# vismaychuriwala/Fast-Image-Editing-with-Generative-Models

Measured on AMD Instinct MI355X. Metric: PIE-Bench images/sec @1024^2 SSD-1B fp16 4-step, higher is better.
Workload: dtype f16

## Files before the change

### fast-image-editing-with-generative-models_amd/csrc/conv_halo.hip

```cpp
#include "gemm_common.h"

using namespace fie_gemm;

namespace {

constexpr int HP = 18;
constexpr int HPIECES = (HP * HP + 7) / 8;
constexpr int HALO_B = HPIECES * 1024;
constexpr int HSLOTS = 6;
constexpr int BNH = 128;
constexpr int STH = 3;
constexpr int WSTAGE_B = BNH * 128;
constexpr int WRING_OFF = 0;
constexpr int HALO_OFF = STH * WSTAGE_B;
constexpr int DUMP_OFF = HALO_OFF + 2 * HALO_B;
constexpr int kLdsHalo = DUMP_OFF + 1024;
constexpr int RWH = BNH / 64;

constexpr int n_w(bool last, int t) { return last && t + 2 > 8 ? 0 : RWH; }
constexpr int n_h(bool last, int t) { return !last && t < HSLOTS ? 1 : 0; }
constexpr int n_wait(bool last, int t) { return (t > 0 ? n_h(last, t - 1) : 0) + n_w(last, t) + n_h(last, t); }

template <bool STAMP>
__global__ __launch_bounds__(512) void conv_halo_kernel(GemmArgs p) {
    constexpr int FM = 4, FN = 4, WM = 64, WN = 64;
    extern __shared__ __attribute__((aligned(16))) half_t smem[];
    char* const lds = reinterpret_cast<char*>(smem);

    const int tid = threadIdx.x;
    const int lane = tid & 63;
    const int wave = __builtin_amdgcn_readfirstlane(tid >> 6);
    const int grp = wave >> 2;
    const int wm = wave & 3, wn = wave >> 2;

    const int bid = xcd_remap(blockIdx.x, gridDim.x);
    const int nt = bid % p.nbn, patch = bid / p.nbn;
    const int ppr = p.OW >> 4, ppi = (p.OH >> 4) * ppr;
    const int b = patch / ppi, pr = patch - b * ppi;
    const int py = pr / ppr, px = pr - py * ppr;
    const int y0 = py << 4, x0 = px << 4;
    const int m0 = (b * p.OH + y0) * p.OW + x0, n0 = nt * BNH;

    const int live = p.probe == 1 ? 0 : 1;
    const __amdgpu_buffer_rsrc_t rs_a = buf_rsrc(p.A1, (int)p.a1_bytes * live);
    const __amdgpu_buffer_rsrc_t rs_w = buf_rsrc(p.Wt, (int)p.w_bytes * live);

    unsigned h_off[HSLOTS];
#pragma unroll
    for (int i = 0; i < HSLOTS; ++i) {
        const int q = wave + 8 * i;
        const int pl = q * 8 + (lane >> 3);
        const int hy = pl / HP, hx = pl - hy * HP;
        const int iy = y0 + hy - 1, ix = x0 + hx - 1;
        const bool ok = q < HPIECES && pl < HP * HP && iy >= 0 && iy < p.H && ix >= 0 && ix < p.W;
        const unsigned chunk = (unsigned)((lane & 7) ^ (hx & 7));
        h_off[i] = ok ? ((unsigned)(b * p.H + iy) * (unsigned)p.W + (unsigned)ix) * (unsigned)p.Cin * 2u + chunk * 16u : kOob;
    }
    auto halo_dst = [&](int i, int buf) -> half_t* {
        const int q = wave + 8 * i;
        return reinterpret_cast<half_t*>(lds + (q < HPIECES ? HALO_OFF + buf * HALO_B + q * 1024 : DUMP_OFF));
    };
    const int lr = lane >> 3;
    const unsigned w_base = (unsigned)(n0 + wave * 8 + lr) * (unsigned)p.ldw * 2u + (unsigned)((lane & 7) ^ lr) * 16u;
    const unsigned w_step = 64u * (unsigned)p.ldw * 2u;
    auto issue_w = [&](int stage, unsigned soff) {
#pragma unroll
        for (int i = 0; i < RWH; ++i)
            bload16(rs_w, reinterpret_cast<half_t*>(lds + WRING_OFF + stage * WSTAGE_B + (wave + 8 * i) * 1024), w_base + (unsigned)i * w_step, soff);
    };
    const unsigned cin2 = (unsigned)p.Cin * 2u;

    const int fr = lane & 15, fq = lane >> 4;
    unsigned a_rd[3][2];
#pragma unroll
    for (int kx = 0; kx < 3; ++kx)
#pragma unroll
        for (int kh = 0; kh < 2; ++kh)
            a_rd[kx][kh] = (unsigned)((wm * FM * HP + fr + kx) * 128 + (((kh * 4 + fq) ^ ((fr + kx) & 7)) << 4));
    unsigned w_rd[2];
#pragma unroll
    for (int kh = 0; kh < 2; ++kh) w_rd[kh] = (unsigned)(2 * lds_off(wn * WN + fr, kh * 4 + fq));

    f32x4 acc[FN][FM];
#pragma unroll
    for (int i = 0; i < FN; ++i)
#pragma unroll
        for (int j = 0; j < FM; ++j) acc[i][j] = (f32x4){0.f, 0.f, 0.f, 0.f};

    unsigned seg[8] = {0, 0, 0, 0, 0, 0, 0, 0}, tprev = 0;
    auto stamp = [&](int i) {
        if constexpr (STAMP) {
            __builtin_amdgcn_sched_barrier(0);
            const unsigned t = (unsigned)__builtin_amdgcn_s_memtime();
            seg[i] += t - tprev;
            tprev = t;
            __builtin_amdgcn_sched_barrier(0);
        }
    };
    if constexpr (STAMP) tprev = (unsigned)__builtin_amdgcn_s_memtime();

    const int nchunks = p.Cin / BK;
#pragma unroll
    for (int i = 0; i < HSLOTS; ++i) bload16(rs_a, halo_dst(i, 0), h_off[i], 0u);
    issue_w(0, 0u);
    issue_w(1, nchunks * 9 > 1 ? cin2 : 0u);
    wait_vm_barrier<RWH>();
    if (grp == 1) __builtin_amdgcn_s_barrier();
    stamp(5);

    f16x8 fw[2][FN], fa[2][FM];
    auto kstep = [&](auto lastc, auto tapc, int c, unsigned hb) {
        constexpr bool LAST = decltype(lastc)::value;
        constexpr int T = decltype(tapc)::value;
        constexpr int KY = T / 3, KX = T % 3;
        constexpr int STAGE = T % STH, FILL = (T + 2) % STH;
        if constexpr (n_w(LAST, T) > 0) {
            constexpr int T2 = (T + 2) % 9;
            const int c2 = T + 2 > 8 ? c + 1 : c;
            issue_w(FILL, (unsigned)T2 * cin2 + (unsigned)c2 * (BK * 2));
        }
        if constexpr (n_h(LAST, T) > 0) bload16(rs_a, halo_dst(T, (c + 1) & 1), h_off[T], (unsigned)(c + 1) * (BK * 2));
        stamp(0);
        const char* const hal = lds + HALO_OFF + hb;
        const char* const wst = lds + WRING_OFF + STAGE * WSTAGE_B;
#pragma unroll
        for (int kh = 0; kh < 2; ++kh) {
#pragma unroll
            for (int i = 0; i < FN; ++i) fw[kh][i] = *reinterpret_cast<const f16x8*>(wst + w_rd[kh] + i * 16 * 128);
#pragma unroll
            for (int j = 0; j < FM; ++j) fa[kh][j] = *reinterpret_cast<const f16x8*>(hal + a_rd[KX][kh] + (j + KY) * HP * 128);
        }
        asm volatile("s_waitcnt lgkmcnt(0)" ::: "memory");
        stamp(1);
        wait_vm_barrier<n_wait(LAST, T)>();
        stamp(2);
        __builtin_amdgcn_sched_barrier(0);
        __builtin_amdgcn_s_setprio(1);
#pragma unroll
        for (int kh = 0; kh < 2; ++kh)
#pragma unroll
            for (int i = 0; i < FN; ++i)
#pragma unroll
                for (int j = 0; j < FM; ++j) acc[i][j] = __builtin_amdgcn_mfma_f32_16x16x32_f16(fw[kh][i], fa[kh][j], acc[i][j], 0, 0, 0);
        __builtin_amdgcn_s_setprio(0);
        __builtin_amdgcn_sched_barrier(0);
        stamp(3);
        __builtin_amdgcn_s_barrier();
        stamp(4);
    };
    auto chunk = [&](auto lastc, int c) {
        const unsigned hb = (c & 1) ? (unsigned)HALO_B : 0u;
        kstep(lastc, std::integral_constant<int, 0>{}, c, hb);
        kstep(lastc, std::integral_constant<int, 1>{}, c, hb);
        kstep(lastc, std::integral_constant<int, 2>{}, c, hb);
        kstep(lastc, std::integral_constant<int, 3>{}, c, hb);
        kstep(lastc, std::integral_constant<int, 4>{}, c, hb);
        kstep(lastc, std::integral_constant<int, 5>{}, c, hb);
        kstep(lastc, std::integral_constant<int, 6>{}, c, hb);
        kstep(lastc, std::integral_constant<int, 7>{}, c, hb);
        kstep(lastc, std::integral_constant<int, 8>{}, c, hb);
    };
    for (int c = 0; c + 1 < nchunks; ++c) chunk(std::false_type{}, c);
    chunk(std::true_type{}, nchunks - 1);
    if (grp == 0) __builtin_amdgcn_s_barrier();

    epilogue<FM, FN, WM, WN, true, true>(p, acc, m0, n0, wm, wn, lane);
    if constexpr (STAMP) {
        asm volatile("s_waitcnt vmcnt(0)" ::: "memory");
        stamp(6);
        if (p.stamps && lane == 0) {
#pragma unroll
            for (int i = 0; i < 8; ++i) p.stamps[((size_t)bid * 8 + wave) * 8 + i] = seg[i];
        }
    }
}


constexpr int K_FIRST = 0, K_MID = 1, K_LAST_F = 2, K_LAST_N = 3, K_LASTREG_S = 4;
constexpr int n2_w(int kind, int t) { return kind == K_LAST_N && t + 2 > 8 ? 0 : RWH; }
constexpr int n2_h(int kind, int t) { return kind != K_LAST_N && t < HSLOTS ? 1 : 0; }
constexpr int n2_st(int var, int kind, int t) { return kind == K_FIRST && t < 8 ? ((var & 2) ? 1 : 2) : 0; }
constexpr int n2_tail(bool res, int kind, int t) { return n2_h(kind, t); }
constexpr int n2_wait(int var, bool res, int kind, int t) {
    return (t > 0 ? n2_tail(res, kind, t - 1) : 0) + ((var & 8) ? 0 : n2_w(kind, t) + n2_tail(res, kind, t));
}
static_assert(n2_tail(true, K_LAST_F, 8) == 0 && n2_tail(true, K_FIRST, 8) == 0 && n2_st(0, K_FIRST, 8) == 0, "tap 8 carries nothing behind its weights");

// ... 587 lines not shown
                }
                su = row16_sum(su);
                sq = row16_sum(sq);
                if (gn_sh >= 3) {
                    float a0 = su, b0 = su, a1 = sq, b1 = sq;
                    asm volatile("s_nop 1\n\tv_permlane16_swap_b32 %0, %1" : "+v"(a0), "+v"(b0));
                    asm volatile("s_nop 1\n\tv_permlane16_swap_b32 %0, %1" : "+v"(a1), "+v"(b1));
                    su = a0 + b0; sq = a1 + b1;
                }
                if (gn_sh >= 4) {
                    float a0 = su, b0 = su, a1 = sq, b1 = sq;
                    asm volatile("s_nop 1\n\tv_permlane32_swap_b32 %0, %1" : "+v"(a0), "+v"(b0));
                    asm volatile("s_nop 1\n\tv_permlane32_swap_b32 %0, %1" : "+v"(a1), "+v"(b1));
                    su = a0 + b0; sq = a1 + b1;
                }
                const int rows_per_group = 1 << (gn_sh - 2);
                const bool ok = fr == 0 && (fq & (rows_per_group - 1)) == 0;
                const unsigned slot = gslot_prev + (unsigned)(JJ * (p.OW >> 4) * p.gn_G) + (unsigned)(((wn * WN + I * 16) >> gn_sh) + (fq >> (gn_sh - 2)));
                u32x2 bits;
                const float2 v2 = make_float2(su, sq);
                __builtin_memcpy(&bits, &v2, 8);
                __builtin_amdgcn_raw_buffer_store_b64(bits, rs_g, ok ? slot * 8u : kOob, 0, 0);
            }, std::make_integer_sequence<int, (FM / 2) * FN>{});
        }
#pragma unroll
        for (int jj = 0; jj < FM / 2; ++jj)
#pragma unroll
            for (int i = 0; i < FN; ++i) {
                u32x4 v = {outp[i][2 * jj][0], outp[i][2 * jj][1], outp[i][2 * jj + 1][0], outp[i][2 * jj + 1][1]};
                if constexpr (DEFER) {
                    asm volatile("s_nop 1\n\tv_permlane16_swap_b32 %0, %1" : "+v"(v[0]), "+v"(v[2]));
                    asm volatile("s_nop 1\n\tv_permlane16_swap_b32 %0, %1" : "+v"(v[1]), "+v"(v[3]));
                }
                __builtin_amdgcn_raw_buffer_store_b128(v, rs_c, edge_off(ro_prev + (unsigned)(2 * jj) * c_jstep + (unsigned)(i * 32), 2 * jj), 0, 0);
            }
    } else {
#pragma unroll
        for (int j = 0; j < FM; ++j)
#pragma unroll
            for (int i = 0; i < FN; ++i) __builtin_amdgcn_raw_buffer_store_b64(outp[i][j], rs_c, ro_prev + (unsigned)j * c_jstep + (unsigned)(i * 32), 0, 0);
    }
    if constexpr (STAMP) {
        asm volatile("s_waitcnt vmcnt(0)" ::: "memory");
        stamp(6);
        if (p.stamps && lane == 0) {
#pragma unroll
            for (int i = 0; i < 8; ++i) p.stamps[((size_t)bid * 8 + wave) * 12 + i] = seg[i];
#pragma unroll
            for (int i = 0; i < 4; ++i) p.stamps[((size_t)bid * 8 + wave) * 12 + 8 + i] = kseg[i];
        }
    }
}

template <bool RES, bool GN, bool RB, int VAR, bool STAMP, bool SIDE = false, bool GNA = false, bool EDGE = false>
hipError_t halo2_attr() {
    return hipFuncSetAttribute(reinterpret_cast<const void*>(&conv_halo2_kernel<RES, GN, RB, VAR, STAMP, SIDE, GNA, EDGE>), hipFuncAttributeMaxDynamicSharedMemorySize, kLdsHalo);
}

}

int fie_conv_halo_init(void) {
    hipError_t e = hipFuncSetAttribute(reinterpret_cast<const void*>(&conv_halo_kernel<false>), hipFuncAttributeMaxDynamicSharedMemorySize, kLdsHalo);
    if (e == hipSuccess) e = hipFuncSetAttribute(reinterpret_cast<const void*>(&conv_halo_kernel<true>), hipFuncAttributeMaxDynamicSharedMemorySize, kLdsHalo);
    if (e == hipSuccess) e = halo2_attr<false, false, false, 6, false>();
    if (e == hipSuccess) e = halo2_attr<false, true, false, 6, false>();
    if (e == hipSuccess) e = halo2_attr<true, false, false, 6, false>();
    if (e == hipSuccess) e = halo2_attr<true, true, false, 6, false>();
    if (e == hipSuccess) e = halo2_attr<false, false, true, 6, false>();
    if (e == hipSuccess) e = halo2_attr<false, true, true, 6, false>();
    if (e == hipSuccess) e = halo2_attr<false, false, false, 0, false>();
    if (e == hipSuccess) e = halo2_attr<false, true, false, 0, false>();
    if (e == hipSuccess) e = halo2_attr<true, false, false, 0, false>();
    if (e == hipSuccess) e = halo2_attr<true, true, false, 0, false>();
    if (e == hipSuccess) e = halo2_attr<false, false, true, 0, false>();
    if (e == hipSuccess) e = halo2_attr<false, true, true, 0, false>();
    if (e == hipSuccess) e = halo2_attr<false, false, false, 6, true>();
    if (e == hipSuccess) e = hipFuncSetAttribute(reinterpret_cast<const void*>(&conv_halo2_kernel<false, false, false, 6, false, true>), hipFuncAttributeMaxDynamicSharedMemorySize, kLdsHalo);
    if (e == hipSuccess) e = hipFuncSetAttribute(reinterpret_cast<const void*>(&conv_halo2_kernel<false, true, false, 6, false, true>), hipFuncAttributeMaxDynamicSharedMemorySize, kLdsHalo);
    if (e == hipSuccess) e = halo2_attr<true, true, false, 6, true>();
    if (e == hipSuccess) e = hipFuncSetAttribute(reinterpret_cast<const void*>(&conv_halo2_kernel<false, true, false, 6, false, false, true>), hipFuncAttributeMaxDynamicSharedMemorySize, kLdsHalo + 8192);
    if (e == hipSuccess) e = hipFuncSetAttribute(reinterpret_cast<const void*>(&conv_halo2_kernel<true, true, false, 6, false, false, true>), hipFuncAttributeMaxDynamicSharedMemorySize, kLdsHalo + 8192);
    if (e == hipSuccess) e = halo2_attr<false, false, false, 6, false, false, false, true>();
    if (e == hipSuccess) e = halo2_attr<true, false, false, 6, false, false, false, true>();
    if (e == hipSuccess) e = halo2_attr<false, false, true, 6, false, false, false, true>();
    if (e == hipSuccess) e = halo2_attr<false, false, false, 6, false, true, false, true>();
    if (e != hipSuccess) {
        fie_set_error("conv_halo: hipFuncSetAttribute failed: %s", hipGetErrorString(e));
        return FIE_EHIP;
    }
    return FIE_OK;
}

bool fie_conv_halo_ok(const GemmArgs& a) {
    const bool base = a.stride == 1 && !a.ups && !a.taps2 && !a.oscat && a.pt == 1 && a.pl == 1 && a.H == a.OH && a.W == a.OW && a.OH % 16 == 0 &&
                      a.OW % 16 == 0 && a.Cin % BK == 0 && a.Cin >= BK && !a.w_scale && !a.out_f8 && a.splitk <= 1;
    if (!base) return false;
    if (!a.A2) return !a.A3 && a.K == 9 * a.Cin;
    return a.C2x % BK == 0 && a.C3x % BK == 0 && a.C2x > 0 && (a.A3 != nullptr) == (a.C3x > 0) && a.K == 9 * a.Cin + a.C2x + a.C3x && a.Cin >= 2 * BK && a.N % BNH == 0 &&
           !a.res && !a.rowbias && a.act == FIE_ACT_NONE && a.scale == 1.f && a.lda2 * 2 * (int64_t)a.OW * a.OH < (1ll << 31) && a.lda3 * 2 * (int64_t)a.OW * a.OH < (1ll << 31);
}

bool fie_conv_halo_edge_ok(const GemmArgs& a) {
    const bool base = a.stride == 1 && !a.ups && !a.taps2 && !a.oscat && a.pt == 1 && a.pl == 1 && a.H == a.OH && a.W == a.OW && a.OH > 0 && a.OW > 0 &&
                      (a.OH % 16 != 0 || a.OW % 16 != 0) && a.M % (a.OH * a.OW) == 0 && a.Cin % BK == 0 && a.Cin >= 2 * BK && !a.w_scale && !a.out_f8 &&
                      a.splitk <= 1 && a.N % 64 == 0 && a.ldc >= a.N && !a.gn_partial && !a.gna_tab && a.act == FIE_ACT_NONE && a.scale == 1.f && !(a.rowbias && a.res);
    if (!base) return false;
    if (!a.A2) return !a.A3 && a.K == 9 * a.Cin;
    return a.C2x % BK == 0 && a.C3x % BK == 0 && a.C2x > 0 && (a.A3 != nullptr) == (a.C3x > 0) && a.K == 9 * a.Cin + a.C2x + a.C3x && !a.res && !a.rowbias &&
           a.lda2 * 2 * (int64_t)a.OW * a.OH < (1ll << 31) && a.lda3 * 2 * (int64_t)a.OW * a.OH < (1ll << 31);
}

int64_t fie_conv_halo_patches(const GemmArgs& a) {
    if (a.OH <= 0 || a.OW <= 0) return 0;
    return (int64_t)(a.M / (a.OH * a.OW)) * ((a.OH + 15) / 16) * ((a.OW + 15) / 16);
}

bool fie_conv_halo_gna_ok(const GemmArgs& a) {
    if (!fie_conv_halo_ok(a) || a.A2 || a.rowbias) return false;
    const int nbn = (a.N + BNH - 1) / BNH;
    return a.M == a.OH * a.OW && a.Cin >= 2 * BK && a.Cin <= 1024 && a.N % BNH == 0 && nbn <= 64 && a.act == FIE_ACT_NONE && a.scale == 1.f && a.gn_partial != nullptr &&
           (a.gn_cg == 4 || a.gn_cg == 8 || a.gn_cg == 16);
}

int fie_launch_conv_halo(fie_ctx* ctx, GemmArgs& a, int variant) {
    if (variant == 6) {
        FIE_REQUIRE(fie_conv_halo_edge_ok(a), "halo-resident conv with edge patches (tile code 78): stride-1 same-size 3x3 conv with H or W %% 16 != 0, Cin %% 64 == 0, "
                    "Cin >= 128, N %% 64 == 0, no activation / scale / GroupNorm sums only");
        a.frag_ld = a.OW;
        a.nbn = (a.N + BNH - 1) / BNH;
        a.nbm = (int)fie_conv_halo_patches(a);
        const int tiles = a.nbm * a.nbn;
        int g = tiles < ctx->num_cus ? tiles : ctx->num_cus;
        g -= g % a.nbn;
        FIE_REQUIRE(g >= a.nbn && a.nbn <= ctx->num_cus, "halo-resident conv: more column tiles than CUs");
        const dim3 grid((unsigned)g);
        if (a.A2) fie_launch(ctx, (conv_halo2_kernel<false, false, false, 6, false, true, false, true>), grid, dim3(512), kLdsHalo, a);
        else if (a.res) fie_launch(ctx, (conv_halo2_kernel<true, false, false, 6, false, false, false, true>), grid, dim3(512), kLdsHalo, a);
        else if (a.rowbias) fie_launch(ctx, (conv_halo2_kernel<false, false, true, 6, false, false, false, true>), grid, dim3(512), kLdsHalo, a);
        else fie_launch(ctx, (conv_halo2_kernel<false, false, false, 6, false, false, false, true>), grid, dim3(512), kLdsHalo, a);
        FIE_LAUNCH_CHECK();
        return FIE_OK;
    }
    FIE_REQUIRE(fie_conv_halo_ok(a), "halo-resident conv: stride-1 same-size 3x3 conv with H, W %% 16 == 0 and Cin %% 64 == 0 only");
    a.frag_ld = a.OW;
    a.nbn = (a.N + BNH - 1) / BNH;
    a.nbm = (a.M / (a.OH * a.OW)) * (a.OH >> 4) * (a.OW >> 4);
    const int tiles = a.nbm * a.nbn;
    const bool side = a.A2 != nullptr;
    FIE_REQUIRE(!(side && variant != 2), "halo-resident conv: 1x1 side inputs run on tile code 72 only");
    if (a.gna_tab) {
        FIE_REQUIRE(fie_conv_halo_gna_ok(a), "halo-resident conv with the input's GroupNorm applied in LDS: shape or epilogue not built (fie_conv3x3_gn_ok)");
        int g = tiles < ctx->num_cus ? tiles : ctx->num_cus;
        g -= g % a.nbn;
        const int lds_bytes = kLdsHalo + a.Cin * 8;
        if (a.res) fie_launch(ctx, (conv_halo2_kernel<true, true, false, 6, false, false, true>), dim3((unsigned)g), dim3(512), lds_bytes, a);
        else fie_launch(ctx, (conv_halo2_kernel<false, true, false, 6, false, false, true>), dim3((unsigned)g), dim3(512), lds_bytes, a);
        FIE_LAUNCH_CHECK();
        return FIE_OK;
    }
    if (!side && variant >= 2 && tiles <= ctx->num_cus) variant = variant == 4 ? 1 : 0;
    if (!side && variant >= 2 && (a.Cin < 2 * BK || a.N % BNH != 0 || (a.rowbias && a.res) || (variant == 4 && a.rowbias) || a.act != FIE_ACT_NONE || a.scale != 1.f)) variant = variant == 4 ? 1 : 0;
    if (variant < 2) {
        const dim3 grid((unsigned)tiles);
        if (variant == 1) fie_launch(ctx, (conv_halo_kernel<true>), grid, dim3(512), kLdsHalo, a);
        else fie_launch(ctx, (conv_halo_kernel<false>), grid, dim3(512), kLdsHalo, a);
        FIE_LAUNCH_CHECK();
        return FIE_OK;
    }
    int g = tiles < ctx->num_cus ? tiles : ctx->num_cus;
    g -= g % a.nbn;
    FIE_REQUIRE(g >= a.nbn && a.nbn <= ctx->num_cus, "halo-resident conv: more column tiles than CUs");
    const dim3 grid((unsigned)g);
    const bool res = a.res != nullptr, gn = a.gn_partial != nullptr, rb = a.rowbias != nullptr;
    FIE_REQUIRE(!gn || a.gn_cg == 4 || a.gn_cg == 8 || a.gn_cg == 16, "halo-resident conv: GroupNorm sums need 4, 8 or 16 channels per group");
#define FIE_HALO2(RES, GN, RB, VAR, ST) fie_launch(ctx, (conv_halo2_kernel<RES, GN, RB, VAR, ST>), grid, dim3(512), kLdsHalo, a)
#define FIE_HALO2_V(VAR)                                                                   \
    do {                                                                                   \
        if (rb && gn) FIE_HALO2(false, true, true, VAR, false);                            \
        else if (rb) FIE_HALO2(false, false, true, VAR, false);                            \
        else if (res && gn) FIE_HALO2(true, true, false, VAR, false);                      \
        else if (res) FIE_HALO2(true, false, false, VAR, false);                           \
        else if (gn) FIE_HALO2(false, true, false, VAR, false);                            \
        else FIE_HALO2(false, false, false, VAR, false);                                   \
    } while (0)
    if (side) { if (gn) fie_launch(ctx, (conv_halo2_kernel<false, true, false, 6, false, true>), grid, dim3(512), kLdsHalo, a); else fie_launch(ctx, (conv_halo2_kernel<false, false, false, 6, false, true>), grid, dim3(512), kLdsHalo, a); }
    else if (variant == 4) { if (res || gn) FIE_HALO2(true, true, false, 6, true); else FIE_HALO2(false, false, false, 6, true); }
    else if (variant == 5) FIE_HALO2_V(0);
    else FIE_HALO2_V(6);
#undef FIE_HALO2_V
#undef FIE_HALO2
    FIE_LAUNCH_CHECK();
    return FIE_OK;
}
```

### fast-image-editing-with-generative-models_amd/csrc/fie_internal.h

```cpp
#pragma once
#include <hip/hip_runtime.h>
#include <stdint.h>
#include <stdio.h>
#include <string.h>
#include <map>
#include <string>
#include <tuple>
#include <utility>
#include <vector>
#include "../../include/fie.h"

typedef _Float16 half_t;
typedef _Float16 f16x8 __attribute__((ext_vector_type(8)));
typedef _Float16 f16x4 __attribute__((ext_vector_type(4)));
typedef _Float16 f16x2 __attribute__((ext_vector_type(2)));
typedef float f32x4 __attribute__((ext_vector_type(4)));
typedef short s16x4 __attribute__((ext_vector_type(4)));
typedef unsigned u32x4 __attribute__((ext_vector_type(4)));

struct fie_launch_rec {
    const void* fn;
    dim3 grid, block;
    unsigned lds;
    std::vector<unsigned char> blob;
// ... 1 lines not shown
};
struct fie_program {
    std::vector<fie_launch_rec> recs;
    hipEvent_t done = nullptr;
    hipStream_t last_stream = nullptr;
    bool has_done = false;
};

struct fie_weight { const void* ptr; int64_t n, ld; };
struct fie_step_cache { char* ptr; int64_t bytes; bool filled; };

struct fie_tile_override { int mode, M, N, K, code; };

struct fie_tune_key {
    int mode, M, N, K, K1, geom, w8;
    bool operator<(const fie_tune_key& o) const {
        return std::tie(mode, M, N, K, K1, geom, w8) < std::tie(o.mode, o.M, o.N, o.K, o.K1, o.geom, o.w8);
    }
};

struct fie_ctx {
    int device;
    hipStream_t stream;
    int num_cus;
    int force_tile = 0;
    int gemm_probe = 0;
    int epi_prefetch = 1;
    unsigned* gemm_stamps = nullptr;
    float* gn_target = nullptr;
    int64_t gn_target_rows = 0;
    int gn_target_groups = 0;
    int attn_variant = 0;
    int gn_onepass = 1;
    unsigned* err_flag = nullptr;
    void* sk_ws = nullptr;
    int64_t sk_bytes = 0;
    int splitk_mode = 1;
    int autotune = 0;
    std::map<fie_tune_key, int> tuned;
    int tune_exclude[16] = {0};
    void* tune_buf = nullptr;
    void* tune_flush = nullptr;
    size_t tune_bytes = 0;
    int n_overrides = 0;
    fie_tile_override overrides[32];
    char last_kernel[128] = "";
    fie_program* recording = nullptr;
    std::vector<std::string>* oplog = nullptr;
    char op_desc[384] = "";
    std::vector<std::string>* tune_cands = nullptr;
    std::map<std::string, fie_program*> graphs;
    std::map<std::string, fie_step_cache> step_caches;
    std::map<std::string, fie_weight> weights;
};

template <typename T>
inline void fie_pack_arg(fie_launch_rec& r, const T& v) {
    size_t off = (r.blob.size() + alignof(T) - 1) / alignof(T) * alignof(T);
    r.blob.resize(off + sizeof(T));
    memcpy(r.blob.data() + off, &v, sizeof(T));
    r.offs.push_back((unsigned)off);
}

void fie_oplog_append(fie_ctx* ctx, const void* fn, dim3 grid, dim3 block, unsigned lds);
#define FIE_DESC(ctx, ...)                                                              \
    do {                                                                                \
        if ((ctx)->oplog) snprintf((ctx)->op_desc, sizeof((ctx)->op_desc), __VA_ARGS__); \
    } while (0)

template <typename... KArgs, typename... Args>
inline void fie_launch(fie_ctx* ctx, void (*kernel)(KArgs...), dim3 grid, dim3 block, unsigned lds, Args&&... args) {
    static_assert(sizeof...(KArgs) == sizeof...(Args), "argument count");
    std::tuple<KArgs...> vals(static_cast<KArgs>(args)...);
    std::apply([&](const KArgs&... a) { hipLaunchKernelGGL(kernel, grid, block, lds, ctx->stream, a...); }, vals);
    if (ctx->oplog) fie_oplog_append(ctx, reinterpret_cast<const void*>(kernel), grid, block, lds);
    if (ctx->recording) {
        fie_launch_rec r;
        r.fn = reinterpret_cast<const void*>(kernel);
        r.grid = grid; r.block = block; r.lds = lds;
        std::apply([&](const KArgs&... a) { (fie_pack_arg(r, a), ...); }, vals);
        ctx->recording->recs.push_back(std::move(r));
    }
}

void fie_set_error(const char* fmt, ...);

#define FIE_REQUIRE(cond, ...)                         \
    do {                                               \
        if (!(cond)) {                                 \
            fie_set_error(__VA_ARGS__);                \
            return FIE_EINVAL;                         \
        }                                              \
    } while (0)

#define FIE_LAUNCH_CHECK()                                                         \
    do {                                                                           \
        hipError_t e__ = hipGetLastError();                                        \
        if (e__ != hipSuccess) {                                                   \
            fie_set_error("%s:%d launch failed: %s", __FILE__, __LINE__,           \
                          hipGetErrorString(e__));                                 \
            return FIE_EHIP;                                                       \
        }                                                                          \
    } while (0)

static inline int64_t fie_roundup(int64_t x, int64_t m) { return (x + m - 1) / m * m; }

// ... 36 lines not shown
```

### fast-image-editing-with-generative-models_amd/hip.py

```python
import ctypes
import os
import subprocess

import torch

from . import header

_CSRC = os.path.join(os.path.dirname(os.path.abspath(__file__)), "csrc")
LIB_PATH = os.environ.get("FIE_LIB_PATH") or os.path.join(_CSRC, "libfie_hip.so")

_P, _I, _F = ctypes.c_void_p, ctypes.c_int, ctypes.c_float

ACT_NONE, ACT_SILU, ACT_GELU, ACT_QUICK_GELU, ACT_GEGLU = (header.DEFINES["ACT_" + n] for n in ("NONE", "SILU", "GELU", "QUICK_GELU", "GEGLU"))
SIGNATURES = {name: args for name, (_, args) in header.FUNCTIONS.items()}

_lib = None


def build(force=False):
    if force:
        subprocess.run(["make", "-C", _CSRC, "clean"], check=True, capture_output=True)
    r = subprocess.run(["make", "-C", _CSRC, "-j4"], capture_output=True, text=True)
    if r.returncode != 0:
        raise RuntimeError("building libfie_hip.so failed:\n" + r.stdout[-4000:] + r.stderr[-4000:])
# ... 76 lines not shown
        assert name in GRAPH_NAMES, name
        _chk(lib().fie_graph_register(self.ctx.h, name.encode(), self.h))

    def close(self):
        if self.h:
            lib().fie_program_destroy(self.ctx.h, self.h)
            self.h = _P()


class W8:

    def __init__(self, q, scale):
        self.q, self.scale = q, scale

    def stride(self, d):
        return self.q.stride(d)

    def dequant(self):
        return self.q.view(torch.float8_e4m3fn).float() * self.scale[:, None]


class Context:

    def __init__(self, device=0, dtype=torch.float16):
        if dtype not in (torch.float16, torch.float32):
            raise ValueError(f"dtype {dtype} not supported (float16 or float32)")
        self.dtype = dtype
        self.f32 = dtype == torch.float32
        if not torch.cuda.is_available():
            raise RuntimeError("no HIP device visible: the fie_amd hot path has no CPU fallback")
        self.device = torch.device("cuda", device)
        h = _P()
        _chk(lib().fie_ctx_create(device, None, ctypes.byref(h)))
        self.h = h
        self._err = torch.zeros(4, device=self.device, dtype=torch.int32)
        self._err_host = torch.zeros(4, dtype=torch.int32).pin_memory()
        _chk(lib().fie_ctx_error_flag(self.h, self._err.data_ptr()))
        self._stream = None
        self._gn_ws = {}
        self._gn_stats = {}
        self._gn_gen = 0
        self._sk_ws = {}
        self._sk_bound = None
        self._sk_pinned = False
        self._cap_stream = None
        self._prog_ws = []
        self.splitk_bytes = int(os.environ.get("FIE_SPLITK_MB", "96")) << 20
        self.gn_from_epilogue = os.environ.get("FIE_GN_FROM_EPILOGUE", "1") != "0"
        self.gn_quads = os.environ.get("FIE_GN_QUADS", "1") != "0"
        self._epi_prefetch = True
        self.up2x_parity = os.environ.get("FIE_UP2X_PARITY", "1") != "0"
        self.ln_fold = os.environ.get("FIE_LN_FOLD", "1") != "0"
        self.kv_group = os.environ.get("FIE_KV_GROUP", "1") != "0"
        self.ln_fold_which = os.environ.get("FIE_LN_FOLD_WHICH", "qkv,q2")
        self.ln_fold_ff1 = os.environ.get("FIE_LN_FOLD_FF1", "0") != "0"
        self.conv_plus_shortcut = os.environ.get("FIE_CONV_PLUS", "1") != "0"
        self._resize_tables = {}
        self.ws_tag = 0
        self._keep = None
        self.w8 = False
        self.a8 = os.environ.get("FIE_A8", "1") != "0"
        self.gn_fuse_conv = os.environ.get("FIE_GN_FUSE_CONV", "0") == "1"
        self.calib = False
        self.tune_frozen = os.environ.get("FIE_TUNE_FROZEN", "0") == "1"
        self.tune_table_entries = 0
        self.load_tune_table()

    def fetch_device_errors(self):
        self._err_host.copy_(self._err, non_blocking=True)

    def check_device_errors(self, fetch=True):
        if fetch:
            self.fetch_device_errors()
            torch.cuda.current_stream(self.device).synchronize()
        code = int(self._err_host[0])
        if code:
            self._err.zero_()
            self._err_host.zero_()
            what = {1: "fie_time_embed_f16: the in-launch barrier timed out (a workgroup never arrived); the timestep embedding of that "
                       "launch is invalid"}.get(code, "unknown device error")
            raise FieError(f"device error {code}: {what}")

    def sync_stream(self):
        s = torch.cuda.current_stream(self.device).cuda_stream
        if s != self._stream:
            _chk(lib().fie_ctx_set_stream(self.h, s))
            self._stream = s

    def load_tune_table(self, path=None):
        path = path or os.environ.get("FIE_TUNE_TABLE")
        if not path or self.f32:
            return 0
        with open(path) as f:
            n = lib().fie_gemm_autotune_load(self.h, f.read().encode())
        if n < 0:
            raise FieError(f"fie_gemm_autotune_load: {lib().fie_last_error().decode()}")
        self.tune_table_entries = n
        return n

    def _bind_splitk(self):
        if self._sk_pinned or self.f32 or not self.splitk_bytes:
            return
        key = (self._stream, self.ws_tag)
        if key == self._sk_bound:
            return
        ws = self._sk_ws.get(key)
# ... 5 lines not shown
    def capture_stream(self):
        if self._cap_stream is None:
            self._cap_stream = torch.cuda.Stream(device=self.device)
        with torch.cuda.stream(self._cap_stream):
            self.sync_stream()
            self._bind_splitk()
        torch.cuda.synchronize(self.device)
        return self._cap_stream

    def splitk_counters_clear(self):
        torch.cuda.synchronize(self.device)
        live = list(self._sk_ws.values()) + [w for w in (r() for r in self._prog_ws) if w is not None]
        return all(int(ws[:16384].view(torch.int32).abs().max()) == 0 for ws in live)

    def record(self):
        import contextlib

        @contextlib.contextmanager
        def cm():
            prog = Program(self)
            self.sync_stream()
            own = None
            if not self.f32 and self.splitk_bytes:
                own = torch.zeros(self.splitk_bytes, device=self.device, dtype=torch.uint8)
                prog.keep.append(own)
                import weakref
                self._prog_ws = [r for r in self._prog_ws if r() is not None] + [weakref.ref(own)]
                _chk(lib().fie_splitk_workspace(self.h, own.data_ptr(), own.numel()))
                self._sk_pinned = True
            _chk(lib().fie_program_begin(self.h, ctypes.byref(prog.h)))
            self._keep = prog.keep
            try:
                yield prog
            finally:
                self._keep = None
                _chk(lib().fie_program_end(self.h))
                if own is not None:
                    self._sk_pinned = False
                    self._sk_bound = None
        return cm()

    def run_named(self, name):
        self.sync_stream()
        _chk(getattr(lib(), "fie_" + name)(self.h))

    def _alloc(self, shape, dtype=None, zero=False):
        t = (torch.zeros if zero else torch.empty)(shape, device=self.device, dtype=dtype or self.dtype)
        if self._keep is not None:
            self._keep.append(t)
        return t

    def force_tile(self, code):
        _chk(lib().fie_debug_force_tile(self.h, int(code)))

    def prefetch(self, t, stream=None, blocks=16):
        _chk(lib().fie_prefetch(self.h, t.data_ptr(), t.numel() * t.element_size(), stream.cuda_stream if stream is not None else None, int(blocks)))

    def autotune(self, on=True):
        _chk(lib().fie_gemm_autotune(self.h, int(on)))

    def tune_exclude(self, codes):
        return lib().fie_debug_tune_exclude(self.h, (codes or "").encode())

    def autotune_report(self):
        buf = ctypes.create_string_buffer(1 << 20)
        n = lib().fie_gemm_autotune_report(self.h, buf, len(buf))
        return n, buf.value.decode()

    def splitk(self, on=True):
        _chk(lib().fie_debug_splitk(self.h, int(bool(on))))

    def oplog(self, on=True):
        _chk(lib().fie_debug_oplog(self.h, int(on)))
        self._oplog_on = bool(on)

    def oplog_mark(self, text):
        if getattr(self, "_oplog_on", False):
            _chk(lib().fie_debug_oplog_mark(self.h, text.encode()))

    def oplog_read(self):
        n = lib().fie_debug_oplog_read(self.h, None, 0)
        buf = ctypes.create_string_buffer(int(n) + 16)
        lib().fie_debug_oplog_read(self.h, buf, len(buf))
        return [l for l in buf.value.decode().split("\n") if l]

    def tune_candidates(self, on=True):
        _chk(lib().fie_debug_tune_candidates(self.h, int(on)))

    def tune_candidates_read(self):
        n = lib().fie_debug_tune_candidates_read(self.h, None, 0)
        buf = ctypes.create_string_buffer(int(n) + 16)
        lib().fie_debug_tune_candidates_read(self.h, buf, len(buf))
        out = []
        for line in buf.value.decode().split("\n"):
            if line:
                key, rest = line.split(" rule=")
                rule, cands = rest.split(" cands=")
                out.append((key, int(rule), [int(c) for c in cands.split(",") if c]))
        return out

    def gemm_stamps(self, buf):
        _chk(lib().fie_debug_gemm_stamps(self.h, buf.data_ptr() if buf is not None else None))

    def gemm_probe(self, mode):
        _chk(lib().fie_debug_gemm_probe(self.h, int(mode)))

# ... 693 lines not shown
```

### include/fie.h

```cpp
#ifndef FIE_H_
#define FIE_H_

#include <stdint.h>

#ifdef __cplusplus
extern "C" {
#endif

#define FIE_OK 0
#define FIE_EINVAL (-1)
#define FIE_EHIP (-2)
#define FIE_ENODEV (-3)

#define FIE_DEVERR_TIME_EMBED_BARRIER 1u

#define FIE_ACT_NONE 0
#define FIE_ACT_SILU 1
#define FIE_ACT_GELU 2
#define FIE_ACT_QUICK_GELU 3
#define FIE_ACT_GEGLU 4

typedef struct fie_ctx fie_ctx;

int fie_version(void);
// ... 173 lines not shown
                           int64_t rows_per_image, int groups, const void* gamma, const void* beta, float eps,
                           int silu, void* workspace);
int fie_layernorm_f32(fie_ctx* ctx, const void* X, int64_t ldx, void* Y, int64_t ldy, int64_t rows, int C,
                      const void* gamma, const void* beta, float eps);
int fie_sinusoid_f32(fie_ctx* ctx, const float* vals, int B, int nvals, int dim, void* out, int64_t ld_out, int col0);
int fie_clip_embed_f32(fie_ctx* ctx, const int32_t* ids, int B, int T, int C, const void* tok_table,
                       const void* pos_table, void* out);
int fie_pixels_in_u8_f32(fie_ctx* ctx, const uint8_t* src, int H, int W, int normalize, void* dst, int copies);
int fie_pixels_out_f32_u8(fie_ctx* ctx, const void* src, int64_t ld_in, int H, int W, uint8_t* dst);
int fie_latent_prep_f32(fie_ctx* ctx, const void* moments, const float* eps_post, const float* noise, int64_t HW,
                        float scaling_factor, float sqrt_ab, float sqrt_1mab, float* latents_out, void* model_in,
                        int copies);
int fie_lcm_step_f32(fie_ctx* ctx, const void* eps, int64_t ld_eps, int nb, float guidance, float* latents,
                     const float* noise, int64_t HW, float sqrt_ab_t, float sqrt_1mab_t, float c_skip, float c_out,
                     float sqrt_ab_prev, float sqrt_1mab_prev, void* model_in, int copies, float inv_scaling,
                     void* decode_in);

int fie_debug_force_tile(fie_ctx* ctx, int tile);
int fie_debug_tile_override(fie_ctx* ctx, const char* spec);
int fie_conv3x3_plus_nhwc_f16(fie_ctx* ctx, const void* X, int B, int H, int W, int Cin, const void* Wpacked, int64_t ldw, void* Y, int64_t ldc, int Cout,
                              const void* bias, const void* rowbias, int64_t ld_rowbias, float scale, int act, const void* X2, int64_t ld2, int C2,
                              const void* X3, int64_t ld3, int C3);

int fie_conv_up2x_nhwc_f16(fie_ctx* ctx, const void* X, int B, int H, int W, int Cin, const void* W4, int64_t ldw, int Npad, void* Y, int64_t ldc,
                           int Cout, const void* bias, const void* rowbias, int64_t ld_rowbias, float scale, int act);

int fie_gn_stats_target(fie_ctx* ctx, void* partial, int64_t rows_per_image, int groups);
int fie_groupnorm_coef_f16(fie_ctx* ctx, int C, int B, int64_t rows_per_image, int groups, const void* gamma, const void* beta, float eps, const void* partial,
                           void* workspace, int partial_groups, float* coef);
int fie_conv3x3_gn_ok(fie_ctx* ctx, int B, int H, int W, int Cin, int Cout, int out_groups);
int fie_conv3x3_gn_nhwc_f16(fie_ctx* ctx, const void* X, int B, int H, int W, int Cin, const float* coef, int silu, const void* Wpacked, int64_t ldw, void* Y,
                            int64_t ldc, int Cout, const void* bias, const void* residual, int64_t ldr);
int64_t fie_gn_stats_bytes(int B, int64_t rows_per_image, int groups);
int fie_groupnorm_stats_nhwc_f16(fie_ctx* ctx, const void* X, int C, void* Y, int B, int64_t rows_per_image, int groups, const void* gamma,
                                 const void* beta, float eps, int silu, const void* partial, void* workspace, int partial_groups);

int fie_prefetch(fie_ctx* ctx, const void* ptr, int64_t bytes, void* stream, int blocks);
int fie_splitk_workspace(fie_ctx* ctx, void* workspace, int64_t bytes);
int fie_debug_splitk(fie_ctx* ctx, int mode);
int fie_gemm_autotune(fie_ctx* ctx, int on);
int fie_gemm_autotune_report(fie_ctx* ctx, char* buf, int cap);
int fie_gemm_autotune_load(fie_ctx* ctx, const char* text);
int fie_debug_tune_exclude(fie_ctx* ctx, const char* codes);
int fie_debug_gemm_probe(fie_ctx* ctx, int mode);
int fie_debug_epilogue_prefetch(fie_ctx* ctx, int on);
int fie_debug_gemm_stamps(fie_ctx* ctx, void* buf);
const char* fie_debug_last_gemm_kernel(fie_ctx* ctx);
int fie_debug_oplog(fie_ctx* ctx, int on);
int fie_debug_oplog_mark(fie_ctx* ctx, const char* text);
int64_t fie_debug_oplog_read(fie_ctx* ctx, char* buf, int64_t cap);
int fie_debug_tune_candidates(fie_ctx* ctx, int on);
int64_t fie_debug_tune_candidates_read(fie_ctx* ctx, char* buf, int64_t cap);
int fie_debug_attn_variant(fie_ctx* ctx, int variant);
int fie_debug_gn_onepass(fie_ctx* ctx, int enable);

int fie_canny_rgb_u8(const uint8_t* rgb, int H, int W, int low, int high, uint8_t* edges_rgb);

int64_t fie_canny_workspace_bytes(int H, int W);
int fie_canny_rgb_device_u8(fie_ctx* ctx, const uint8_t* rgb, int H, int W, int low, int high, void* workspace,
                            uint8_t* edges_rgb, int* iterations);
int fie_canny_rgb_device_begin_u8(fie_ctx* ctx, const uint8_t* rgb, int H, int W, int low, int high, int rounds, void* workspace, uint8_t* edges_rgb,
                                  int* host_flags);
int fie_canny_rgb_device_finish_u8(fie_ctx* ctx, int H, int W, void* workspace, uint8_t* edges_rgb, int* host_flags, int* iterations);

int fie_resize_rgb_u8(fie_ctx* ctx, const uint8_t* src, int H, int W, uint8_t* dst, int OH, int OW, const int* kx,
                      const int* bx, int ksx, const int* ky, const int* by, int ksy, uint8_t* tmp);

int fie_resize_l_u8(fie_ctx* ctx, const uint8_t* src, int H, int W, uint8_t* dst, int OH, int OW, const int* kx,
                    const int* bx, int ksx, const int* ky, const int* by, int ksy, uint8_t* tmp);

int fie_mask_prep(fie_ctx* ctx, const uint8_t* mask_l, int H, int W, const float* taps, int radius, float* mask_px,
                  uint8_t* mask_lat);
int fie_latent_prep_src(fie_ctx* ctx, const void* moments, const float* eps_post, const float* noise, int64_t HW,
                        float scaling_factor, float sqrt_ab, float sqrt_1mab, float* latents_out, void* model_in,
                        int copies, float* z0_out);
int fie_latent_prep_src_f32(fie_ctx* ctx, const void* moments, const float* eps_post, const float* noise, int64_t HW,
                            float scaling_factor, float sqrt_ab, float sqrt_1mab, float* latents_out, void* model_in,
                            int copies, float* z0_out);
int fie_lcm_step_masked(fie_ctx* ctx, const void* eps, int64_t ld_eps, int nb, float guidance, float* latents,
                        const float* noise, int64_t HW, float sqrt_ab_t, float sqrt_1mab_t, float c_skip, float c_out,
                        float sqrt_ab_prev, float sqrt_1mab_prev, void* model_in, int copies, float inv_scaling,
                        void* decode_in, const uint8_t* mask_lat, const float* z0, const float* noise_init);
int fie_lcm_step_masked_f32(fie_ctx* ctx, const void* eps, int64_t ld_eps, int nb, float guidance, float* latents,
                            const float* noise, int64_t HW, float sqrt_ab_t, float sqrt_1mab_t, float c_skip, float c_out,
                            float sqrt_ab_prev, float sqrt_1mab_prev, void* model_in, int copies, float inv_scaling,
                            void* decode_in, const uint8_t* mask_lat, const float* z0, const float* noise_init);
int fie_pixels_out_composite_f16_u8(fie_ctx* ctx, const void* src, int64_t ld_in, int H, int W, const uint8_t* source,
                                    const float* mask, uint8_t* dst);
int fie_pixels_out_composite_f32_u8(fie_ctx* ctx, const void* src, int64_t ld_in, int H, int W, const uint8_t* source,
                                    const float* mask, uint8_t* dst);

#define FIE_CONTENT_ORIGINAL 0
#define FIE_CONTENT_FILL 1
#define FIE_CONTENT_LATENT_NOISE 2
#define FIE_CONTENT_LATENT_NOTHING 3
int64_t fie_mask_fill_workspace_bytes(int H, int W);
int fie_mask_fill_rgb_u8(fie_ctx* ctx, const uint8_t* src, const uint8_t* mask_l, int H, int W, void* workspace, uint8_t* out,
                         const uint8_t* ctl_in, uint8_t* ctl_out);
int fie_latent_prep_src_content(fie_ctx* ctx, const void* moments, const float* eps_post, const float* noise, int64_t HW,
                                float scaling_factor, float sqrt_ab, float sqrt_1mab, float* latents_out, void* model_in,
                                int copies, float* z0_out, const uint8_t* mask_lat, int mode);
int fie_latent_prep_src_content_f32(fie_ctx* ctx, const void* moments, const float* eps_post, const float* noise, int64_t HW,
                                    float scaling_factor, float sqrt_ab, float sqrt_1mab, float* latents_out, void* model_in,
                                    int copies, float* z0_out, const uint8_t* mask_lat, int mode);

int64_t fie_multiband_workspace_bytes(int H, int W, int levels);
// ... 36 lines not shown
```

Baseline: 15.50.

## Add selectable halo conv tile forms (16x16x160, 8x16x160) chosen by wave-quantization cost

Templates the halo-resident 3x3 conv kernel on patch height and output-channel tile width. This adds 16x16x160 and 8x16x160 forms alongside the original 16x16x128. A rule picks the form that minimizes per-CU wave cost when the 128-wide tiling gives too few tiles for the CUs, or when N is not a multiple of 128. The aim is to reduce tail/underfill waste on small-grid convs such as 320/640/1280-channel layers. A debug override and env var are added, and the non-multiple-of-8 weight pieces go to a dump slot, which adds extra instantiations and some wasted loads.

```diff
diff --git a/fast-image-editing-with-generative-models_amd/csrc/conv_halo.hip b/fast-image-editing-with-generative-models_amd/csrc/conv_halo.hip
--- a/fast-image-editing-with-generative-models_amd/csrc/conv_halo.hip
+++ b/fast-image-editing-with-generative-models_amd/csrc/conv_halo.hip
@@ -1,4 +1,5 @@
 #include "gemm_common.h"
+#include "halo_form.h"
 
 using namespace fie_gemm;
 
@@ -17,13 +18,32 @@
 constexpr int kLdsHalo = DUMP_OFF + 1024;
 constexpr int RWH = BNH / 64;
 
-constexpr int n_w(bool last, int t) { return last && t + 2 > 8 ? 0 : RWH; }
-constexpr int n_h(bool last, int t) { return !last && t < HSLOTS ? 1 : 0; }
-constexpr int n_wait(bool last, int t) { return (t > 0 ? n_h(last, t - 1) : 0) + n_w(last, t) + n_h(last, t); }
-
-template <bool STAMP>
+template <int PH, int BN>
+struct HaloTile {
+    static_assert((PH == 16 || PH == 8) && (BN == 128 || BN == 160), "forms 1..3 of halo_form.h");
+    static constexpr int FM = PH / 4, FN = BN / 32;
+    static constexpr int HPY = PH + 2;
+    static constexpr int PIECES = (HPY * HP + 7) / 8;
+    static constexpr int HALO = PIECES * 1024;
+    static constexpr int SLOTS = (PIECES + 7) / 8;
+    static constexpr int WSTAGE = BN * 128;
+    static constexpr int WPIECES = BN / 8;
+    static constexpr int RW = (WPIECES + 7) / 8;
+    static constexpr int HALO_OFF = STH * WSTAGE;
+    static constexpr int DUMP_OFF = HALO_OFF + 2 * HALO;
+    static constexpr int LDS = DUMP_OFF + 1024;
+    static_assert(2 * WSTAGE + (FN - 1) * 2048 < 65536 && LDS <= 160 * 1024, "ds_read_b128 offset field; LDS of a CU");
+    static constexpr int n_w(bool last, int t) { return last && t + 2 > 8 ? 0 : RW; }
+    static constexpr int n_h(bool last, int t) { return !last && t < SLOTS ? 1 : 0; }
+    static constexpr int n_wait(bool last, int t) { return (t > 0 ? n_h(last, t - 1) : 0) + n_w(last, t) + n_h(last, t); }
+};
+static_assert(HaloTile<16, 128>::LDS == kLdsHalo && HaloTile<16, 128>::SLOTS == HSLOTS && HaloTile<16, 128>::RW == RWH && HaloTile<16, 128>::HALO == HALO_B, "form 1 is the persistent kernel's layout");
+
+template <int PH, int BN, bool STAMP>
 __global__ __launch_bounds__(512) void conv_halo_kernel(GemmArgs p) {
-    constexpr int FM = 4, FN = 4, WM = 64, WN = 64;
+    using T = HaloTile<PH, BN>;
+    constexpr int FM = T::FM, FN = T::FN, WM = FM * 16, WN = FN * 16;
+    constexpr int HSLOTS = T::SLOTS, HPIECES = T::PIECES, HALO_B = T::HALO, HALO_OFF = T::HALO_OFF, DUMP_OFF = T::DUMP_OFF, WSTAGE_B = T::WSTAGE, RWH = T::RW;
     extern __shared__ __attribute__((aligned(16))) half_t smem[];
     char* const lds = reinterpret_cast<char*>(smem);
 
@@ -35,11 +55,11 @@
 
     const int bid = xcd_remap(blockIdx.x, gridDim.x);
     const int nt = bid % p.nbn, patch = bid / p.nbn;
-    const int ppr = p.OW >> 4, ppi = (p.OH >> 4) * ppr;
+    const int ppr = p.OW >> 4, ppi = (p.OH >> (PH == 16 ? 4 : 3)) * ppr;
     const int b = patch / ppi, pr = patch - b * ppi;
     const int py = pr / ppr, px = pr - py * ppr;
-    const int y0 = py << 4, x0 = px << 4;
-    const int m0 = (b * p.OH + y0) * p.OW + x0, n0 = nt * BNH;
+    const int y0 = py << (PH == 16 ? 4 : 3), x0 = px << 4;
+    const int m0 = (b * p.OH + y0) * p.OW + x0, n0 = nt * BN;
 
     const int live = p.probe == 1 ? 0 : 1;
     const __amdgpu_buffer_rsrc_t rs_a = buf_rsrc(p.A1, (int)p.a1_bytes * live);
@@ -52,7 +72,7 @@
         const int pl = q * 8 + (lane >> 3);
         const int hy = pl / HP, hx = pl - hy * HP;
         const int iy = y0 + hy - 1, ix = x0 + hx - 1;
-        const bool ok = q < HPIECES && pl < HP * HP && iy >= 0 && iy < p.H && ix >= 0 && ix < p.W;
+        const bool ok = q < HPIECES && pl < T::HPY * HP && iy >= 0 && iy < p.H && ix >= 0 && ix < p.W;
         const unsigned chunk = (unsigned)((lane & 7) ^ (hx & 7));
         h_off[i] = ok ? ((unsigned)(b * p.H + iy) * (unsigned)p.W + (unsigned)ix) * (unsigned)p.Cin * 2u + chunk * 16u : kOob;
     }
@@ -65,8 +85,14 @@
     const unsigned w_step = 64u * (unsigned)p.ldw * 2u;
     auto issue_w = [&](int stage, unsigned soff) {
 #pragma unroll
-        for (int i = 0; i < RWH; ++i)
-            bload16(rs_w, reinterpret_cast<half_t*>(lds + WRING_OFF + stage * WSTAGE_B + (wave + 8 * i) * 1024), w_base + (unsigned)i * w_step, soff);
+        for (int i = 0; i < RWH; ++i) {
+            if constexpr (T::WPIECES % 8 == 0) {
+                bload16(rs_w, reinterpret_cast<half_t*>(lds + WRING_OFF + stage * WSTAGE_B + (wave + 8 * i) * 1024), w_base + (unsigned)i * w_step, soff);
+            } else {
+                const bool piece = wave + 8 * i < T::WPIECES;
+                bload16(rs_w, reinterpret_cast<half_t*>(lds + (piece ? WRING_OFF + stage * WSTAGE_B + (wave + 8 * i) * 1024 : DUMP_OFF)), piece ? w_base + (unsigned)i * w_step : kOob, soff);
+            }
+        }
     };
     const unsigned cin2 = (unsigned)p.Cin * 2u;
 
@@ -111,15 +137,15 @@
     f16x8 fw[2][FN], fa[2][FM];
     auto kstep = [&](auto lastc, auto tapc, int c, unsigned hb) {
         constexpr bool LAST = decltype(lastc)::value;
-        constexpr int T = decltype(tapc)::value;
-        constexpr int KY = T / 3, KX = T % 3;
-        constexpr int STAGE = T % STH, FILL = (T + 2) % STH;
-        if constexpr (n_w(LAST, T) > 0) {
-            constexpr int T2 = (T + 2) % 9;
-            const int c2 = T + 2 > 8 ? c + 1 : c;
+        constexpr int TAP = decltype(tapc)::value;
+        constexpr int KY = TAP / 3, KX = TAP % 3;
+        constexpr int STAGE = TAP % STH, FILL = (TAP + 2) % STH;
+        if constexpr (T::n_w(LAST, TAP) > 0) {
+            constexpr int T2 = (TAP + 2) % 9;
+            const int c2 = TAP + 2 > 8 ? c + 1 : c;
             issue_w(FILL, (unsigned)T2 * cin2 + (unsigned)c2 * (BK * 2));
         }
-        if constexpr (n_h(LAST, T) > 0) bload16(rs_a, halo_dst(T, (c + 1) & 1), h_off[T], (unsigned)(c + 1) * (BK * 2));
+        if constexpr (T::n_h(LAST, TAP) > 0) bload16(rs_a, halo_dst(TAP, (c + 1) & 1), h_off[TAP], (unsigned)(c + 1) * (BK * 2));
         stamp(0);
         const char* const hal = lds + HALO_OFF + hb;
         const char* const wst = lds + WRING_OFF + STAGE * WSTAGE_B;
@@ -132,7 +158,7 @@
         }
         asm volatile("s_waitcnt lgkmcnt(0)" ::: "memory");
         stamp(1);
-        wait_vm_barrier<n_wait(LAST, T)>();
+        wait_vm_barrier<T::n_wait(LAST, TAP)>();
         stamp(2);
         __builtin_amdgcn_sched_barrier(0);
         __builtin_amdgcn_s_setprio(1);
@@ -826,6 +852,16 @@
     }
 }
 
+template <int PH, int BN, bool STAMP>
+hipError_t halo1_attr() {
+    return hipFuncSetAttribute(reinterpret_cast<const void*>(&conv_halo_kernel<PH, BN, STAMP>), hipFuncAttributeMaxDynamicSharedMemorySize, HaloTile<PH, BN>::LDS);
+}
+
+template <int PH, int BN, bool STAMP>
+void halo1_launch(fie_ctx* ctx, const GemmArgs& a) {
+    fie_launch(ctx, (conv_halo_kernel<PH, BN, STAMP>), dim3((unsigned)(a.nbm * a.nbn)), dim3(512), HaloTile<PH, BN>::LDS, a);
+}
+
 template <bool RES, bool GN, bool RB, int VAR, bool STAMP, bool SIDE = false, bool GNA = false, bool EDGE = false>
 hipError_t halo2_attr() {
     return hipFuncSetAttribute(reinterpret_cast<const void*>(&conv_halo2_kernel<RES, GN, RB, VAR, STAMP, SIDE, GNA, EDGE>), hipFuncAttributeMaxDynamicSharedMemorySize, kLdsHalo);
@@ -834,8 +870,12 @@
 }
 
 int fie_conv_halo_init(void) {
-    hipError_t e = hipFuncSetAttribute(reinterpret_cast<const void*>(&conv_halo_kernel<false>), hipFuncAttributeMaxDynamicSharedMemorySize, kLdsHalo);
-    if (e == hipSuccess) e = hipFuncSetAttribute(reinterpret_cast<const void*>(&conv_halo_kernel<true>), hipFuncAttributeMaxDynamicSharedMemorySize, kLdsHalo);
+    hipError_t e = halo1_attr<16, 128, false>();
+    if (e == hipSuccess) e = halo1_attr<16, 128, true>();
+    if (e == hipSuccess) e = halo1_attr<16, 160, false>();
+    if (e == hipSuccess) e = halo1_attr<16, 160, true>();
+    if (e == hipSuccess) e = halo1_attr<8, 160, false>();
+    if (e == hipSuccess) e = halo1_attr<8, 160, true>();
     if (e == hipSuccess) e = halo2_attr<false, false, false, 6, false>();
     if (e == hipSuccess) e = halo2_attr<false, true, false, 6, false>();
     if (e == hipSuccess) e = halo2_attr<true, false, false, 6, false>();
@@ -935,9 +975,20 @@
     if (!side && variant >= 2 && tiles <= ctx->num_cus) variant = variant == 4 ? 1 : 0;
     if (!side && variant >= 2 && (a.Cin < 2 * BK || a.N % BNH != 0 || (a.rowbias && a.res) || (variant == 4 && a.rowbias) || a.act != FIE_ACT_NONE || a.scale != 1.f)) variant = variant == 4 ? 1 : 0;
     if (variant < 2) {
-        const dim3 grid((unsigned)tiles);
-        if (variant == 1) fie_launch(ctx, (conv_halo_kernel<true>), grid, dim3(512), kLdsHalo, a);
-        else fie_launch(ctx, (conv_halo_kernel<false>), grid, dim3(512), kLdsHalo, a);
+        const int images = a.M / (a.OH * a.OW);
+        const int form = ctx->halo_form ? ctx->halo_form : variant == 1 ? 1 : halo_form_choose(images, a.OH, a.OW, a.N, ctx->num_cus);
+        FIE_REQUIRE(halo_form_fits(form, a.N), "halo-resident conv: form %d (%d x 16 patch x %d channels, fie_debug_halo_form) takes N %% %d == 0 only (N = %d)", form,
+                    halo_form_ph(form), halo_form_bn(form), halo_form_bn(form), a.N);
+        a.nbn = (a.N + halo_form_bn(form) - 1) / halo_form_bn(form);
+        a.nbm = images * (a.OH / halo_form_ph(form)) * (a.OW >> 4);
+        if (form == 2) { if (variant == 1) halo1_launch<16, 160, true>(ctx, a); else halo1_launch<16, 160, false>(ctx, a); }
+        else if (form == 3) { if (variant == 1) halo1_launch<8, 160, true>(ctx, a); else halo1_launch<8, 160, false>(ctx, a); }
+        else if (variant == 1) halo1_launch<16, 128, true>(ctx, a);
+        else halo1_launch<16, 128, false>(ctx, a);
+        if (form != 1) {
+            char* const at = strstr(ctx->last_kernel, "<256x128>");
+            if (at) memcpy(at, form == 2 ? "<256x160>" : "<128x160>", 9);
+        }
         FIE_LAUNCH_CHECK();
         return FIE_OK;
     }
@@ -966,3 +1017,9 @@
     FIE_LAUNCH_CHECK();
     return FIE_OK;
 }
+
+extern "C" int fie_debug_halo_form(fie_ctx* ctx, int form) {
+    FIE_REQUIRE(ctx != nullptr && form >= 0 && form <= kHaloForms, "fie_debug_halo_form: 0 = by rule, 1 = 16x16x128, 2 = 16x16x160, 3 = 8x16x160");
+    ctx->halo_form = form;
+    return FIE_OK;
+}
diff --git a/fast-image-editing-with-generative-models_amd/csrc/fie_internal.h b/fast-image-editing-with-generative-models_amd/csrc/fie_internal.h
--- a/fast-image-editing-with-generative-models_amd/csrc/fie_internal.h
+++ b/fast-image-editing-with-generative-models_amd/csrc/fie_internal.h
@@ -77,6 +77,7 @@
     std::map<std::string, fie_program*> graphs;
     std::map<std::string, fie_step_cache> step_caches;
     std::map<std::string, fie_weight> weights;
+    int halo_form = 0;
 };
 
 template <typename T>
diff --git a/fast-image-editing-with-generative-models_amd/csrc/halo_form.h b/fast-image-editing-with-generative-models_amd/csrc/halo_form.h
--- /dev/null
+++ b/fast-image-editing-with-generative-models_amd/csrc/halo_form.h
@@ -0,0 +1,28 @@
+#pragma once
+#include <stdint.h>
+
+namespace fie_gemm {
+
+constexpr int kHaloForms = 3;
+constexpr int halo_form_ph(int form) { return form == 3 ? 8 : 16; }
+constexpr int halo_form_bn(int form) { return form == 1 ? 128 : 160; }
+
+constexpr bool halo_form_fits(int form, int N) { return form == 1 || (form >= 2 && form <= kHaloForms && N > 0 && N % 160 == 0); }
+
+constexpr int64_t halo_form_tiles(int form, int images, int OH, int OW, int N) {
+    return (int64_t)images * (OH / halo_form_ph(form)) * (OW / 16) * ((N + halo_form_bn(form) - 1) / halo_form_bn(form));
+}
+
+constexpr int64_t halo_form_cost(int form, int images, int OH, int OW, int N, int cus) {
+    return (halo_form_tiles(form, images, OH, OW, N) + cus - 1) / cus * (halo_form_ph(form) * 16 * halo_form_bn(form));
+}
+
+constexpr int halo_form_choose(int images, int OH, int OW, int N, int cus) {
+    if (N % 128 == 0 && halo_form_tiles(1, images, OH, OW, N) > cus) return 1;
+    int best = 1;
+    for (int f = 2; f <= kHaloForms; ++f)
+        if (halo_form_fits(f, N) && halo_form_cost(f, images, OH, OW, N, cus) < halo_form_cost(best, images, OH, OW, N, cus)) best = f;
+    return best;
+}
+
+}
diff --git a/fast-image-editing-with-generative-models_amd/hip.py b/fast-image-editing-with-generative-models_amd/hip.py
--- a/fast-image-editing-with-generative-models_amd/hip.py
+++ b/fast-image-editing-with-generative-models_amd/hip.py
@@ -152,6 +152,8 @@
         self.up2x_parity = os.environ.get("FIE_UP2X_PARITY", "1") != "0"
         self.ln_fold = os.environ.get("FIE_LN_FOLD", "1") != "0"
         self.kv_group = os.environ.get("FIE_KV_GROUP", "1") != "0"
+        if os.environ.get("FIE_HALO_FORM", "0") != "0":
+            self.halo_form(int(os.environ["FIE_HALO_FORM"]))
         self.ln_fold_which = os.environ.get("FIE_LN_FOLD_WHICH", "qkv,q2")
         self.ln_fold_ff1 = os.environ.get("FIE_LN_FOLD_FF1", "0") != "0"
         self.conv_plus_shortcut = os.environ.get("FIE_CONV_PLUS", "1") != "0"
@@ -263,6 +265,9 @@
 
     def force_tile(self, code):
         _chk(lib().fie_debug_force_tile(self.h, int(code)))
+
+    def halo_form(self, form):
+        _chk(lib().fie_debug_halo_form(self.h, int(form)))
 
     def prefetch(self, t, stream=None, blocks=16):
         _chk(lib().fie_prefetch(self.h, t.data_ptr(), t.numel() * t.element_size(), stream.cuda_stream if stream is not None else None, int(blocks)))
diff --git a/include/fie.h b/include/fie.h
--- a/include/fie.h
+++ b/include/fie.h
@@ -249,6 +249,7 @@
 int fie_debug_tune_candidates(fie_ctx* ctx, int on);
 int64_t fie_debug_tune_candidates_read(fie_ctx* ctx, char* buf, int64_t cap);
 int fie_debug_attn_variant(fie_ctx* ctx, int variant);
+int fie_debug_halo_form(fie_ctx* ctx, int form);
 int fie_debug_gn_onepass(fie_ctx* ctx, int enable);
 
 int fie_canny_rgb_u8(const uint8_t* rgb, int H, int W, int low, int high, uint8_t* edges_rgb);
```

Measured after the change: 15.45. No clear change (-0.3%).
